# gchq/annchor

Hardware: AMD Instinct MI355X
Metric: knn_graph_builds_per_s (1 / Annchor.fit() wall-clock; BASELINE: k-NN graph build time + recall@k) (higher is better)
Workload: dtype int32 bit-vectors (Levenshtein) + f64 (bounds/regression/selection); 1 GPU; load_strings Levenshtein N=1600 n_anchors=15 k=25 p_work=0.12 niters=2; parallelism=one GPU

## Files before the change

annchor_amd/_native.py:

```python
import ctypes
import os

import numpy as np

_HERE = os.path.dirname(os.path.abspath(__file__))
LIB_PATH = os.environ.get("ANNCHOR_HIP_LIB", os.path.join(_HERE, "libannchor_hip.so"))

F_D, F_A, F_SID, F_IJS, F_I_PTR, F_I_IDX, F_FEATURES, F_NCM, F_RA, F_LABELS, F_THRESH, F_PROB, F_CAND, F_NEXT, F_DAD = range(1, 16)
_FIELD_DTYPE = {
    F_D: np.float64, F_A: np.int64, F_SID: np.uint64, F_IJS: np.int64, F_I_PTR: np.int64, F_I_IDX: np.int64,
    F_FEATURES: np.float64, F_NCM: np.uint8, F_RA: np.float64, F_LABELS: np.int64, F_THRESH: np.float64,
    F_PROB: np.float64, F_CAND: np.int64, F_NEXT: np.int64, F_DAD: np.float64,
}

METRIC_LEVENSHTEIN, METRIC_EUCLIDEAN_F32, METRIC_EUCLIDEAN_F64, METRIC_WASSERSTEIN = 1, 2, 3, 4
METRIC_COSINE_F32, METRIC_COSINE_F64 = 5, 6
METRIC_DTW_F32, METRIC_DTW_F64 = 7, 8
METRIC_FRECHET_F32, METRIC_FRECHET_F64 = 9, 10
METRIC_HAUSDORFF_F32, METRIC_HAUSDORFF_F64 = 11, 12
METRIC_ERP_F32, METRIC_ERP_F64 = 13, 14
METRIC_EMD_POINTS_F32, METRIC_EMD_POINTS_F64 = 15, 16
METRIC_JACCARD_TOKENS, METRIC_JACCARD_BITS = 17, 18
METRIC_WEIGHTED_LEVENSHTEIN = 19
METRIC_MSM_F32, METRIC_MSM_F64 = 20, 21
# ... 71 lines not shown
    "annchor_legacy_generate": (ctypes.c_int, [ctypes.c_uint32, _i64]),
    "annchor_legacy_generate_at_next_wait": (ctypes.c_int, [_vp, ctypes.c_uint32, _i64, _i64]),
    "annchor_legacy_choice_ranks": (ctypes.c_int, [ctypes.c_uint32, _vp, _vp, _i32, _vp, _vp]),
    "annchor_legacy_choice_begin": (ctypes.c_int, [ctypes.c_uint32, _vp, _vp, _i32, ctypes.POINTER(_vp)]),
    "annchor_legacy_choice_end": (ctypes.c_int, [_vp, _vp, _vp]),
    "annchor_ols_bins": (ctypes.c_int, [_vp, _vp, _vp, _i64, _i32, _vp, _i32, _vp, _vp, _vp, _vp]),
    "annchor_gather_features": (ctypes.c_int, [_vp, _vp, _i64, _vp]),
    "annchor_evaluate_samples": (ctypes.c_int, [_vp, _vp, _i64, _vp]),
    "annchor_set_samples": (ctypes.c_int, [_vp, _vp, _i64, _vp]),
    "annchor_predict_merge": (ctypes.c_int, [_vp, _vp, _i32, _vp, _vp, _i32, _i32, _vp]),
    "annchor_merge_host_prediction": (ctypes.c_int, [_vp, _vp, _i32, _i32]),
    "annchor_set_labels": (ctypes.c_int, [_vp, _vp]),
    "annchor_select_candidates": (ctypes.c_int, [_vp, _i32, _i32, _vp, _vp, _i32, _i64, _i32,
                                                 ctypes.POINTER(_i64), ctypes.POINTER(_i64)]),
    "annchor_select_prepare": (ctypes.c_int, [_vp, _i32, _i32]),
    "annchor_mark_candidates": (ctypes.c_int, [_vp]),
    "annchor_refine_candidates": (ctypes.c_int, [_vp]),
    "annchor_park_refine": (ctypes.c_int, [_vp, _i32]),
    "annchor_set_refined": (ctypes.c_int, [_vp, _vp, _i64]),
    "annchor_update_bounds": (ctypes.c_int, [_vp]),
    "annchor_update_bounds_prepare": (ctypes.c_int, [_vp]),
    "annchor_overlap_stats": (ctypes.c_int, [_vp, _vp]),
    "annchor_neighbor_graph": (ctypes.c_int, [_vp, _i32, _vp, _vp]),
    "annchor_stream_bind": (ctypes.c_int, [_vp, _vp, _i64, _i32, _i64, _i32]),
    "annchor_stream_anchor_round": (ctypes.c_int, [_vp, _vp, _i32, _i32, ctypes.POINTER(_dbl), ctypes.POINTER(_i64)]),
    "annchor_stream_get_row": (ctypes.c_int, [_vp, _i64, _vp]),
    "annchor_stream_order": (ctypes.c_int, [_vp, _i32] + [ctypes.POINTER(_vp)] * 6 + [ctypes.POINTER(_i64), ctypes.POINTER(_i32),
                                                                                   ctypes.POINTER(_i32)]),
    "annchor_stream_knn": (ctypes.c_int, [_vp, _vp, _vp, _vp, _vp, _vp, _vp, _i64, _i32, _i32, _i32, _i32, _i32, _i32, _dbl, _i32, _i32, _vp,
                                          _vp, _vp, ctypes.POINTER(_i64)]),
# ... 630 lines not shown
        if errs_list is None:
            self._chk(self.lib.annchor_select_candidates(self.h, int(n_neighbors), int(nmin), None, None, int(n_labels), int(n_refine),
                                                         int(lookahead), ctypes.byref(nc), ctypes.byref(nn)))
            return nc.value, nn.value
        ptr = np.zeros(len(errs_list) + 1, dtype=np.int64)
        np.cumsum([len(e) for e in errs_list], out=ptr[1:])
        errs = _c(np.concatenate(errs_list) if len(errs_list) else np.zeros(0), np.float64)
        self._chk(self.lib.annchor_select_candidates(self.h, int(n_neighbors), int(nmin), _ptr(errs), _ptr(ptr),
                                                     len(errs_list), int(n_refine), int(lookahead),
                                                     ctypes.byref(nc), ctypes.byref(nn)))
        return nc.value, nn.value

    def select_prepare(self, n_neighbors, nmin):
        self._chk(self.lib.annchor_select_prepare(self.h, int(n_neighbors), int(nmin)))

    def mark_candidates(self):
        self._chk(self.lib.annchor_mark_candidates(self.h))

    def refine_candidates(self):
        self._chk(self.lib.annchor_refine_candidates(self.h))

    def park_refine(self, action):
        self._chk(self.lib.annchor_park_refine(self.h, int(action)))

    def set_refined(self, exact):
        exact = _c(exact, np.float64)
        self._chk(self.lib.annchor_set_refined(self.h, _ptr(exact), len(exact)))

    def update_bounds(self):
        self._chk(self.lib.annchor_update_bounds(self.h))
# ... 393 lines not shown
```

annchor_amd/csrc/common.h:

```cpp
#pragma once
#include <hip/hip_runtime.h>

#include <cstdint>
#include <cstdio>
#include <cstring>
#include <string>
#include <vector>
#include <chrono>

#include "../../include/annchor_hip.h"

#define ANN_WAVE 64

struct DevBuf {
    void *p = nullptr;
    size_t cap = 0;
    bool in_arena = false;
    template <typename T> T *as() const { return reinterpret_cast<T *>(p); }
};

struct ProfEntry {
    const char *name;
    double ms = 0;
    int64_t launches = 0;
// ... 127 lines not shown

    DevBuf thresh;
    DevBuf cand, next;
    int64_t ncand = 0, nnext = 0;
    bool cand_marked = false;
    DevBuf gl_val, gl_pos, gl_cnt, gl_ncomp, marked, markcount;
    DevBuf gn_state;
    bool sel_prepared = false;
    int sel_k = 0, sel_nmin = 0;
    bool gn_pending = false;
    int gn_round = 0, gn_L = 0;
    DevBuf sel_hist, sel_state, blk_cnt, blk_off;
    DevBuf sel_pass_state;
    DevBuf tie_lists, tie_hist;
    const void *tie_hist_clean = nullptr;
    DevBuf sel2, sel_bufA, sel_bufB, sel_seg;
    const void *sel2_clean = nullptr;
    DevBuf errs, errptr;
    DevBuf ecdf_index;
    DevBuf cptr, cidx, cval;
    DevBuf c16, cbnd;
    DevBuf tmp0, tmp1, tmp2, tmp3;
    DevBuf scan_tmp;

    DevBuf stage_in, stage_out;

    bool prof_on = false;
    int prof_mode = 0;
    std::vector<hipEvent_t> ev_pool;
    std::vector<ProfEntry> prof;
// ... 30 lines not shown

#define ANN_REQUIRE(c, cond, code, ...)    \
    do {                                   \
        if (!(cond)) {                     \
            ann_set_err((c), __VA_ARGS__); \
            return (code);                 \
        }                                  \
    } while (0)

int ann_reserve(annchor_ctx *c, DevBuf &b, size_t bytes);
int ann_arena_init(annchor_ctx *c, int64_t nx);
int ann_prewarm_state(annchor_ctx *c);
void ann_lev_ap_probe(annchor_ctx *c);
size_t ann_sel2_table_bytes();
size_t ann_tie_hist_bytes();
size_t ann_sel_state_bytes();
int ann_h2d(annchor_ctx *c, void *dst, const void *src, size_t bytes);
hipError_t ann_sync(annchor_ctx *c, const char *where);
int ann_dev_alloc(annchor_ctx *c, void **p, size_t want, size_t *got);
void ann_dev_free(annchor_ctx *c, void *p, size_t bytes);
struct Sel2Epilogue;
int ann_kth_async(annchor_ctx *c, const double *vals, const uint8_t *flag, int64_t n, const int64_t *ks, int nk,
                  const unsigned long long **d_prefix, const int **d_unfinished, const Sel2Epilogue *epi = nullptr);
void ann_kth_async_done(annchor_ctx *c);
int ann_d2h(annchor_ctx *c, void *dst, const void *src, size_t bytes);
int ann_d2h_then(annchor_ctx *c, void *dst, const void *src, size_t bytes, int (*then)(annchor_ctx *));
int ann_d2h2(annchor_ctx *c, void *dst1, const void *src1, size_t bytes1, void *dst2, const void *src2, size_t bytes2);

int ann_prof_entry(annchor_ctx *c, const char *name);
struct ProfGroup {
// ... 180 lines not shown
```

annchor_amd/csrc/ctx.hip:

```cpp
#include <cstdarg>
#include <cmath>
#include <cstdlib>

#include "common.h"
#include <algorithm>
#include <chrono>
#include <mutex>

static std::string g_create_err;
void ann_stream_release(annchor_ctx *c);
void ann_enemies_release(annchor_ctx *c);
void ann_draw_forget(annchor_ctx *c);
void ann_comm_release(annchor_ctx *c);
hipError_t ann_comm_guarded_sync(annchor_ctx *c, hipStream_t stream, const char *where);

const char *ann_set_err(annchor_ctx *c, const char *fmt, ...)
{
    char buf[1024];
    va_list ap;
    va_start(ap, fmt);
    vsnprintf(buf, sizeof buf, fmt, ap);
    va_end(ap);
    if (c && c->comm_aborted && c->err.rfind("collective timed out", 0) == 0) return c->err.c_str();
    if (c) c->err = buf; else g_create_err = buf;
// ... 135 lines not shown
    size_t got = 0;
    if ((p = pool_take(c->device, bytes, &got)) != nullptr) bytes = got;
    else if (hipMalloc(&p, bytes) != hipSuccess) { (void)hipGetLastError(); return ANNCHOR_OK; }
    c->arena = (char *)p;
    c->arena_size = bytes;
    c->arena_off = 0;
    return ANNCHOR_OK;
}

int ann_prewarm_state(annchor_ctx *c)
{
    if (!c->arena || c->state_prewarmed) return ANNCHOR_OK;
    const size_t slot_bytes = sizeof(unsigned long long) * 4 * 1024 + 64;
    struct Piece { DevBuf *b; size_t bytes; };
    Piece pieces[] = {{&c->dev_flags, sizeof(int32_t) * 16}, {&c->lev_cursors, 4 * sizeof(int32_t)}, {&c->sel_state, ann_sel_state_bytes()},
                      {&c->sel2, ann_sel2_table_bytes()},    {&c->tie_hist, ann_tie_hist_bytes()},   {&c->lev_ap, slot_bytes}};
    size_t need = 0;
    for (auto &q : pieces) {
        if (q.b->p) return ANNCHOR_OK;
        need += (q.bytes + 255) & ~(size_t)255;
    }
    if (c->arena_off + need > c->arena_size) return ANNCHOR_OK;
    char *first = c->arena + c->arena_off;
    for (auto &q : pieces) ANN_TRY(ann_reserve(c, *q.b, q.bytes));
    ANN_CHECK_HIP(c, hipMemsetAsync(first, 0, need, c->stream));
    c->dev_flags_clean = true;
    c->lev_cursor_epoch = 0;
    c->gn_err_clean = true;
    c->sel2_clean = c->sel2.p;
    c->tie_hist_clean = c->tie_hist.p;
    c->lev_ap_epoch = 0;
    c->state_prewarmed = true;
    return ANNCHOR_OK;
}

int ann_h2d(annchor_ctx *c, void *dst, const void *src, size_t bytes)
{
    if (bytes == 0) return ANNCHOR_OK;
    if (c->pin && bytes <= annchor_ctx::PIN_SLOT_BYTES) {
        const int sl = c->pin_next;
        c->pin_next = (sl + 1) % annchor_ctx::PIN_SLOTS;
        if (c->pin_busy[sl]) ANN_CHECK_HIP(c, hipEventSynchronize(c->pin_ev[sl]));
        unsigned char *slot = c->pin + (size_t)sl * annchor_ctx::PIN_SLOT_BYTES;
        memcpy(slot, src, bytes);
        ANN_CHECK_HIP(c, hipMemcpyAsync(dst, slot, bytes, hipMemcpyHostToDevice, c->stream));
// ... 1157 lines not shown
```

annchor_amd/csrc/select.hip:

```cpp
#include "common.h"
#include "rowsel.h"
#include "selstate.h"

__global__ __launch_bounds__(ROW_THREADS) void k_row_thresh(const int64_t *__restrict__ Iptr, RowSrc src, uint32_t k,
                                                           double *__restrict__ thresh, int cap)
{
    __shared__ RowSelShared sh;
    __shared__ RowCand rc;
    extern __shared__ __attribute__((aligned(16))) unsigned char dyn_rt[];
    uint64_t *keys = reinterpret_cast<uint64_t *>(dyn_rt);
    const int64_t i = row_of_block(gridDim.x);
    const int64_t b = Iptr[i];
    const int len = (int)(Iptr[i + 1] - b);
    if (len <= 0) { if (threadIdx.x == 0) thresh[i] = -INFINITY; return; }
    const RowView rv = row_view(src, i, b);
    const uint32_t kk = k >= (uint32_t)len ? (uint32_t)len - 1 : k;
    {
        const int cnt = row_candidates(rc, len, (int)kk + 1, [&](int s) { return row_key_asc(rv.val(s)); }, [](int) { return true; },
                                       [](int, uint64_t, bool) {});
        const int cnts = cnt > (int)kk ? row_cand_shrink(rc, cnt, (int)kk + 1, src.shrink_min) : -1;
        if (cnts > (int)kk) {
            for (int e = threadIdx.x; e < cnts; e += ROW_THREADS) {
                const uint64_t ke = rc.key[e];
                uint32_t less = 0, leq = 0;
// ... 490 lines not shown
    const int k0 = threadIdx.x * per, k1 = min(k0 + per, ix.nb + 1);
    uint32_t mine = 0;
    for (int k = k0; k < k1; ++k) mine += T[k];
    csum[threadIdx.x] = mine;
    __syncthreads();
    if (threadIdx.x == 0) {
        uint32_t run = 0;
        for (int q = 0; q < 256; ++q) { const uint32_t v = csum[q]; csum[q] = run; run += v; }
        index[b] = ix;
    }
    __syncthreads();
    uint32_t run = csum[threadIdx.x];
    for (int k = k0; k < k1; ++k) { run += T[k]; T[k] = run; }
}

__global__ __launch_bounds__(256) void k_prob(int64_t n, const int2 *__restrict__ ij, const double *__restrict__ thresh,
                                             const double *__restrict__ RA, const uint8_t *__restrict__ ncm,
                                             const uint8_t *__restrict__ label, const double *__restrict__ errs,
                                             const int64_t *__restrict__ errptr, int nlabels, int lds_cap_entries,
                                             double *__restrict__ prob, int stream, const EcdfIndex *__restrict__ index,
                                             const uint32_t *__restrict__ table)
{
    extern __shared__ __attribute__((aligned(16))) unsigned char dyn[];
    double *le = reinterpret_cast<double *>(dyn);
    __shared__ int64_t lptr[257];
    __shared__ EcdfIndex lix[256];
    for (int t = threadIdx.x; t <= nlabels; t += blockDim.x) lptr[t] = errptr[t];
    if (index)
        for (int t = threadIdx.x; t < nlabels; t += blockDim.x) lix[t] = index[t];
    __syncthreads();
    const bool errs_in_lds = lptr[nlabels] <= (int64_t)lds_cap_entries;
    if (errs_in_lds) {
        const int64_t tot = lptr[nlabels];
        for (int64_t t = threadIdx.x; t < tot; t += blockDim.x) le[t] = errs[t];
        __syncthreads();
    }
    const double *E = errs_in_lds ? le : errs;
    constexpr int PI = 8;
    const int64_t stride = (int64_t)gridDim.x * blockDim.x * PI;
    for (int64_t p0 = (int64_t)blockIdx.x * blockDim.x * PI + threadIdx.x; p0 < n; p0 += stride) {
        uint8_t m[PI], lbv[PI];
        int2 q[PI];
        double ra[PI];
#pragma unroll
        for (int e = 0; e < PI; ++e) {
            const int64_t p = p0 + (int64_t)e * blockDim.x;
            const bool in = p < n;
            const int64_t pc = in ? p : 0;
            m[e] = ann_load(ncm + pc, stream);
            const long long qq = ann_load(reinterpret_cast<const long long *>(ij) + pc, stream);
            q[e] = make_int2((int)(qq & 0xffffffffll), (int)(qq >> 32));
// ... 19 lines not shown
                hi[e] = b[e] + (int32_t)t1;
                lo[e] = b[e] + (int32_t)t0;
            }
            busy |= lo[e] < hi[e];
        }
        while (busy) {
            busy = false;
#pragma unroll
            for (int e = 0; e < PI; ++e)
                if (lo[e] < hi[e]) {
                    const int32_t mid = (lo[e] + hi[e]) >> 1;
                    if (E[mid] < pv[e]) lo[e] = mid + 1; else hi[e] = mid;
                    busy |= lo[e] < hi[e];
                }
        }
#pragma unroll
        for (int e = 0; e < PI; ++e) {
            const int64_t p = p0 + (int64_t)e * blockDim.x;
            if (p >= n) continue;
            double pr = -1.0;
            if (m[e]) {
                if ((int)lbv[e] < nlabels) {
                    const int32_t len = (int32_t)lptr[lbv[e] + 1] - b[e];
                    pr = (double)(lo[e] - b[e]) / (double)len;
                } else {
                    pr = 0.0;
                }
            }
            ann_store(prob + p, pr, stream);
        }
    }
}

#define CP_THREADS 256
#define CP_ITEMS 8
#define CP_SUBTILE (CP_THREADS * CP_ITEMS)
static inline int cp_nsub(int64_t n) { return n >= (16ll << 20) ? 4 : 1; }


#define TIE_CAP 65536

__host__ __device__ __forceinline__ unsigned long long ann_tie_scramble(int64_t p)
{
    return ((unsigned long long)p * 0x9E3779B97F4A7C15ull) >> 11;
}

// ... 34 lines not shown
#pragma unroll
    for (int off = 32; off > 0; off >>= 1) {
        g1 += __shfl_xor(g1, off); g5 += __shfl_xor(g5, off); n1 += __shfl_xor(n1, off); n5 += __shfl_xor(n5, off);
    }
    if ((threadIdx.x & 63) == 0) { atomicAdd(&acc[0], g1); atomicAdd(&acc[1], g5); atomicAdd(&acc[2], n1); atomicAdd(&acc[3], n5); }
    __syncthreads();
    for (int t = threadIdx.x; t < 2 * TIE_BINS; t += 256) {
        const uint32_t c = (&h[0][0])[t];
        if (c) atomicAdd(&ghist[t], c);
    }
    if (threadIdx.x == 0) {
        if (acc[0]) atomicAdd((unsigned long long *)&cs->tie_gt1, acc[0]);
        if (acc[1]) atomicAdd((unsigned long long *)&cs->tie_gt5, acc[1]);
        if (acc[2]) atomicAdd((unsigned long long *)&cs->tie_n1, acc[2]);
        if (acc[3]) atomicAdd((unsigned long long *)&cs->tie_n5, acc[3]);
    }
}

__global__ __launch_bounds__(1024) void k_tie_pick(CutState *__restrict__ cs, uint32_t *__restrict__ ghist)
{
    __shared__ unsigned long long wsum[16];
    const int lane = threadIdx.x & 63, wave = threadIdx.x >> 6;
    for (int q = 0; q < 2; ++q) {
        const bool all = q == 0 ? cs->all1 : cs->all5;
        const long long cnt = q == 0 ? cs->tie_n1 : cs->tie_n5;
        const long long e = q == 0 ? cs->K1 - cs->tie_gt1 : cs->K5 - cs->tie_gt5;
        uint32_t *h = ghist + q * TIE_BINS;
        constexpr int PER = TIE_BINS / 1024;
        unsigned long long c[PER], mine = 0;
#pragma unroll
// ... 467 lines not shown
        for (int q = 0; q < GN_BATCH; ++q, ++round)
            k_gn_round<<<ann_blocks(nx * 64, 256), 256, 0, c->stream>>>(
                nx, nmin, L, Lw, c->gl_val.as<double>(), oth, twin, c->gl_cnt.as<int32_t>(), c->gl_ncomp.as<int32_t>(),
                masks[round & 1], masks[(round + 1) & 1], mout[round % 3], mout[(round + 1) % 3], mout[(round + 2) % 3],
                changed + q, gn_err_ptr(c));
    }
    k_gn_apply<<<ann_blocks(nx * L, 256), 256, 0, c->stream>>>(nx, L, Lw, c->gl_pos.as<int32_t>(), c->gl_cnt.as<int32_t>(),
                                                              masks[round & 1], c->RA.as<double>());
    ANN_CHECK_HIP(c, hipGetLastError());
    c->gn_pending = false;
    return ANNCHOR_OK;
}

size_t ann_tie_hist_bytes() { return sizeof(uint32_t) * 2 * TIE_BINS; }

extern "C" int annchor_select_prepare(annchor_ctx *c, int32_t n_neighbors, int32_t nmin)
{
    if (!c) return ANNCHOR_EINVAL;
    ANN_REQUIRE(c, c->have_RA, ANNCHOR_EINVAL, "RefineApprox not initialised");
    ANN_REQUIRE(c, n_neighbors >= 1 && nmin >= 0, ANNCHOR_EINVAL, "bad selection parameters");
    ANN_CHECK_HIP(c, hipSetDevice(c->device));
    ANN_TRY(select_stage_a(c, n_neighbors, nmin));
    c->sel_prepared = true; c->sel_k = n_neighbors; c->sel_nmin = nmin;
    return ANNCHOR_OK;
}

extern "C" int annchor_select_candidates(annchor_ctx *c, int32_t n_neighbors, int32_t nmin, const double *errs,
                                         const int64_t *err_ptr, int32_t nlabels, int64_t n_refine, int32_t lookahead,
                                         int64_t *n_cand, int64_t *n_next)
{
// ... 9 lines not shown
            ANN_REQUIRE(c, err_ptr[b + 1] > err_ptr[b], ANNCHOR_ESTATE, "error bin %d has no samples", b);
    ANN_CHECK_HIP(c, hipSetDevice(c->device));
    const int64_t n = c->n, nx = c->nx;
    if (!(c->sel_prepared && c->sel_k == n_neighbors && c->sel_nmin == nmin)) ANN_TRY(select_stage_a(c, n_neighbors, nmin));
    c->sel_prepared = false;
    ANN_TRY(select_stage_finish(c));
    (void)nx;
    const int64_t nerr = dev_errs ? 2 * c->nsamp + 64 : err_ptr[nlabels];
    if (!dev_errs) {
        ANN_TRY(ann_reserve(c, c->errs, sizeof(double) * (size_t)nerr));
        ANN_TRY(ann_reserve(c, c->errptr, sizeof(int64_t) * (size_t)(MAXBINS > nlabels ? MAXBINS + 1 : nlabels + 1)));
        ANN_TRY(ann_h2d(c, c->errs.p, errs, sizeof(double) * (size_t)nerr));
        ANN_TRY(ann_h2d(c, c->errptr.p, err_ptr, sizeof(int64_t) * (size_t)(nlabels + 1)));
        c->errs_on_device = false; c->model_cache_valid = false;
    }
    {
        const int64_t lds_entries = dev_errs ? c->nsamp + 64 : nerr;
        const int in_lds = lds_entries * 8 <= 60 * 1024;
        const size_t dyn = in_lds ? (size_t)lds_entries * 8 : 0;
        int blocks = min(ann_blocks(n, 256 * 8), c->prop.multiProcessorCount * 8);
        ProfScope ps(c, "ecdf_probability", (double)n * 26.0);
        static const long long index_min = getenv("ANNCHOR_ECDF_INDEX_MIN") ? atoll(getenv("ANNCHOR_ECDF_INDEX_MIN")) : (4ll << 20);
        EcdfIndex *index = nullptr;
        uint32_t *table = nullptr;
        if (n >= index_min && nlabels > 0 && nerr > 0 && nerr < (1ll << 29)) {
            const size_t idx_bytes = (sizeof(EcdfIndex) * (size_t)nlabels + 15) & ~(size_t)15;
            ANN_TRY(ann_reserve(c, c->ecdf_index, idx_bytes + sizeof(uint32_t) * (size_t)(2 * nerr + nlabels + 1)));
            index = c->ecdf_index.as<EcdfIndex>();
            table = reinterpret_cast<uint32_t *>(c->ecdf_index.as<char>() + idx_bytes);
            k_ecdf_index<<<nlabels, 256, 0, c->stream>>>(c->errs.as<double>(), c->errptr.as<int64_t>(), index, table);
        }
        k_prob<<<blocks, 256, dyn, c->stream>>>(n, c->ij.as<int2>(), c->thresh.as<double>(), c->RA.as<double>(),
                                               c->ncm.as<uint8_t>(), c->label.as<uint8_t>(), c->errs.as<double>(),
                                               c->errptr.as<int64_t>(), nlabels, in_lds ? (int)lds_entries : 0, c->prob.as<double>(), n >= ANN_STREAM_MIN_PAIRS,
                                               index, table);
    }
    ANN_CHECK_HIP(c, hipGetLastError());
    int64_t n_unc = 0;
    ANN_TRY(annchor_count_uncomputed(c, &n_unc));
    CutState cs;
    memset(&cs, 0, sizeof cs);
    cs.K1 = n_refine;
    cs.K5 = n_refine * (int64_t)lookahead;
    cs.all1 = n_refine >= n_unc;
    cs.all5 = cs.all1 || cs.K5 >= n_unc;
    cs.t1 = cs.t5 = INFINITY;
    const unsigned long long *d_cut_prefix = nullptr;
    const int *d_cut_unfinished = nullptr;
    int64_t cut_ks[2];
    int cut_nk = 0;
// ... 8 lines not shown
    if (cs.all1) cs.t1 = -1.0;
    if (cs.all5) cs.t5 = -1.0;
    if (n_refine == 0) { cs.all1 = cs.all5 = 0; cs.t1 = cs.t5 = INFINITY; cs.K1 = cs.K5 = 0; }
    const int nsub = cp_nsub(n);
    const int nb = ann_blocks(n, (int64_t)CP_SUBTILE * nsub);
    ANN_TRY(ann_reserve(c, c->sel_state, SEL_STATE_BYTES));
    ANN_TRY(ann_reserve(c, c->blk_cnt, sizeof(uint32_t) * 4 * (size_t)nb));
    ANN_TRY(ann_reserve(c, c->blk_off, sizeof(int64_t) * 4 * (size_t)nb));
    const int64_t maxc = cs.all1 ? n_unc : cs.K1, maxn = cs.all5 ? n_unc : cs.K5;
    ANN_TRY(ann_reserve(c, c->cand, sizeof(int32_t) * (size_t)(maxc + 1)));
    ANN_TRY(ann_reserve(c, c->next, sizeof(int32_t) * (size_t)(maxn + 1)));
    cs.rk1 = cs.rk5 = ~0ull;
    if (n_refine > 0 && !(cs.all1 && cs.all5)) {
        if (!cs.all1) cut_ks[cut_nk++] = n_unc - cs.K1;
        if (!cs.all5) cut_ks[cut_nk++] = n_unc - cs.K5;
        if (!getenv("ANNCHOR_CUT_WAIT")) {
            Sel2Epilogue ep;
            memset(&ep, 0, sizeof ep);
            ep.kind = 2; ep.cs = c->sel_state.as<CutState>(); ep.cs_init = cs; ep.need1 = !cs.all1; ep.need5 = !cs.all5;
            ep.force_redo = getenv("ANNCHOR_CUT_FORCE_REDO") ? 1 : 0;
            ANN_TRY(ann_kth_async(c, c->prob.as<double>(), c->ncm.as<uint8_t>(), n, cut_ks, cut_nk, &d_cut_prefix, &d_cut_unfinished, &ep));
        }
        if (!d_cut_prefix) ANN_TRY(cut_values_waiting());
    }
    const CutState cs_in = cs;
    if (!d_cut_prefix) ANN_TRY(ann_h2d(c, c->sel_state.p, &cs, sizeof cs));
    const bool ties = n_refine > 0 && !(cs.all1 && cs.all5);
    ANN_TRY(ann_reserve(c, c->tie_lists, sizeof(unsigned long long) * 2 * TIE_CAP));
    unsigned long long *tl1 = c->tie_lists.as<unsigned long long>(), *tl5 = tl1 + TIE_CAP;
    auto split = [&]() {
        ProfScope ps(c, "topk_split_compact", (double)n * 16.0 + (double)(maxc + maxn) * 4.0);
        k_cut_count<<<nb, CP_THREADS, 0, c->stream>>>(c->prob.as<double>(), c->RA.as<double>(), n, c->sel_state.as<CutState>(),
                                                     c->blk_cnt.as<uint32_t>(), nsub);
        k_cut_scan<<<1, CS_THREADS, 0, c->stream>>>(c->blk_cnt.as<uint32_t>(), nb, c->sel_state.as<CutState>(), c->blk_off.as<int64_t>());
        k_cut_emit<<<nb, CP_THREADS, 0, c->stream>>>(c->prob.as<double>(), c->RA.as<double>(), n, c->sel_state.as<CutState>(),
                                                    c->blk_off.as<int64_t>(), c->cand.as<int32_t>(), c->next.as<int32_t>(), nsub);
    };
    auto tie_groups = [&]() -> int {
        ProfScope ps(c, "topk_tie_groups", (double)n * 8.0);
        const int tb = (int)std::min<int64_t>(ann_blocks(n, 256 * TIE_U), (int64_t)c->prop.multiProcessorCount * 3);
        const char *cap_env = getenv("ANNCHOR_TIE_CAP");
        const long long cap = cap_env ? std::min<long long>(TIE_CAP, std::max<long long>(1, atoll(cap_env))) : TIE_CAP;
        ANN_TRY(ann_reserve(c, c->tie_hist, sizeof(uint32_t) * 2 * TIE_BINS));
        if (c->tie_hist_clean != c->tie_hist.p) {
            ANN_CHECK_HIP(c, hipMemsetAsync(c->tie_hist.p, 0, sizeof(uint32_t) * 2 * TIE_BINS, c->stream));
            c->tie_hist_clean = c->tie_hist.p;
        }
        k_tie_hist<<<tb, 256, 0, c->stream>>>(c->prob.as<double>(), n, c->sel_state.as<CutState>(), c->tie_hist.as<uint32_t>());
        k_tie_pick<<<1, 1024, 0, c->stream>>>(c->sel_state.as<CutState>(), c->tie_hist.as<uint32_t>());
        k_tie_collect<<<tb, 256, 0, c->stream>>>(c->prob.as<double>(), n, c->sel_state.as<CutState>(), tl1, tl5, cap);
        k_tie_select<<<1, 1024, 0, c->stream>>>(c->sel_state.as<CutState>(), tl1, tl5, cap);
        return ANNCHOR_OK;
    };
    if (ties) ANN_TRY(tie_groups());
    split();
    ANN_CHECK_HIP(c, hipEventRecord(c->call_b, c->stream));
    c->call_timed = true;
    ANN_CHECK_HIP(c, hipGetLastError());
    if (nmin > 0) {
        unsigned char both[SEL_ERR_OFF + 4];
        ANN_TRY(ann_d2h(c, both, c->sel_state.p, sizeof both));
        int32_t e = 0;
        memcpy(&cs, both, sizeof cs);
        memcpy(&e, both + SEL_ERR_OFF, 4);
        c->gn_err_clean = e == 0;
        ANN_REQUIRE(c, e == 0, ANNCHOR_ESTATE, "guarantee_nmin: a row has fewer not-computed candidates than it must refine");
    } else {
        ANN_TRY(ann_d2h(c, &cs, c->sel_state.p, sizeof cs));
    }
    if (d_cut_prefix) {
        ann_kth_async_done(c);
        if (cs.sel_unfinished) {
            cs = cs_in;
            ANN_TRY(cut_values_waiting());
            ANN_TRY(ann_h2d(c, c->sel_state.p, &cs, sizeof cs));
            if (ties) ANN_TRY(tie_groups());
            split();
            ANN_CHECK_HIP(c, hipGetLastError());
            ANN_TRY(ann_d2h(c, &cs, c->sel_state.p, sizeof cs));
        }
    }
    if (cs.tie_overflow) {
        ANN_TRY(ann_reserve(c, c->marked, (size_t)n));
        for (int q = 0; q < 2; ++q) {
            const bool all = q == 0 ? cs.all1 : cs.all5;
            const int64_t cnt = q == 0 ? cs.tie_n1 : cs.tie_n5, e = q == 0 ? cs.K1 - cs.tie_gt1 : cs.K5 - cs.tie_gt5;
            unsigned long long rk = ~0ull;
            if (!all && e < cnt) {
                if (e <= 0) rk = 0ull;
                else {
                    ANN_TRY(ann_reserve(c, c->colT, sizeof(double) * (size_t)n));
// ... 106 lines not shown
```

include/annchor_hip.h:

```cpp
#ifndef ANNCHOR_HIP_H
#define ANNCHOR_HIP_H

#include <stdint.h>

#ifdef __cplusplus
extern "C" {
#endif

typedef struct annchor_ctx annchor_ctx;

enum {
    ANNCHOR_OK = 0,
    ANNCHOR_EINVAL = -1,
    ANNCHOR_EHIP = -2,
    ANNCHOR_ENODEV = -3,
    ANNCHOR_ELIMIT = -4,
    ANNCHOR_ESTATE = -5
};

enum { ANNCHOR_METRIC_NONE = 0, ANNCHOR_METRIC_LEVENSHTEIN = 1, ANNCHOR_METRIC_EUCLIDEAN_F32 = 2,
       ANNCHOR_METRIC_EUCLIDEAN_F64 = 3, ANNCHOR_METRIC_WASSERSTEIN = 4, ANNCHOR_METRIC_COSINE_F32 = 5,
       ANNCHOR_METRIC_COSINE_F64 = 6, ANNCHOR_METRIC_DTW_F32 = 7, ANNCHOR_METRIC_DTW_F64 = 8,
       ANNCHOR_METRIC_FRECHET_F32 = 9, ANNCHOR_METRIC_FRECHET_F64 = 10, ANNCHOR_METRIC_HAUSDORFF_F32 = 11,
       ANNCHOR_METRIC_HAUSDORFF_F64 = 12, ANNCHOR_METRIC_ERP_F32 = 13, ANNCHOR_METRIC_ERP_F64 = 14,
// ... 132 lines not shown
                                     uint32_t seed, int64_t *n_out, int32_t *taken);
int annchor_legacy_choice_ranks_device(annchor_ctx *ctx, uint32_t seed, const int64_t *counts, const int64_t *want, int32_t nbins,
                                       int64_t *ranks_out, int32_t *taken);
int annchor_download_samples(annchor_ctx *ctx, int64_t *positions, double *feats, double *sample_y, double *sample_predict);
int annchor_fit_regression_device(annchor_ctx *ctx, const double *bins, int32_t nbins, int32_t first_iteration, int32_t is_metric);
int annchor_fit_errors_device(annchor_ctx *ctx);
int annchor_model_download(annchor_ctx *ctx, double *W, double *c, int32_t *status, int64_t *err_ptr, int32_t *flags );
int annchor_errors_download(annchor_ctx *ctx, double *errs, int64_t n_errs);
int annchor_model_download_with_errors(annchor_ctx *ctx, double *W, double *c, int32_t *status, int64_t *err_ptr, int32_t *flags ,
                                       double *errs, int64_t errs_cap, int64_t *n_errs);

int annchor_select_candidates(annchor_ctx *ctx, int32_t n_neighbors, int32_t nmin, const double *errs,
                              const int64_t *err_ptr, int32_t nlabels, int64_t n_refine,
                              int32_t lookahead, int64_t *n_cand, int64_t *n_next);
int annchor_select_prepare(annchor_ctx *ctx, int32_t n_neighbors, int32_t nmin);
int annchor_mark_candidates(annchor_ctx *ctx);
int annchor_refine_candidates(annchor_ctx *ctx);
int annchor_lev_persist_state(int set);

int annchor_park_refine(annchor_ctx *ctx, int32_t action);
int annchor_set_refined(annchor_ctx *ctx, const double *exact, int64_t n_cand);

int annchor_update_bounds(annchor_ctx *ctx);
int annchor_update_bounds_prepare(annchor_ctx *ctx);
int annchor_overlap_stats(annchor_ctx *ctx, int64_t *out);

int annchor_neighbor_graph(annchor_ctx *ctx, int32_t n_neighbors, int64_t *ng_idx, double *ng_dist);

int annchor_stream_bind(annchor_ctx *ctx, const float *X, int64_t n_local, int32_t dim, int64_t global_base,
                        int32_t x_on_device);
// ... 107 lines not shown
```

Baseline: 388.1 graphs/s.

## Derive probability cut thresholds from a fused per-key count table

The probability kernel now builds a per-block shared-memory histogram over the discrete (label, ECDF rank) keys that every probability value maps to, and merges it into a small global table. A single-block kernel then finds the k-th largest cut values and tie-group counts from this table. This replaces the separate async k-th selection pass over all pair probabilities, and a reduced-pass tie histogram follows it. It adds atomic work and LDS pressure to k_prob and falls back to the old path when the table overflows or its totals do not match.

```diff
diff --git a/annchor_amd/_native.py b/annchor_amd/_native.py
--- a/annchor_amd/_native.py
+++ b/annchor_amd/_native.py
@@ -109,6 +109,7 @@
     "annchor_select_candidates": (ctypes.c_int, [_vp, _i32, _i32, _vp, _vp, _i32, _i64, _i32,
                                                  ctypes.POINTER(_i64), ctypes.POINTER(_i64)]),
     "annchor_select_prepare": (ctypes.c_int, [_vp, _i32, _i32]),
+    "annchor_cut_stats": (ctypes.c_int, [_vp, ctypes.POINTER(_i64), ctypes.POINTER(_i64)]),
     "annchor_mark_candidates": (ctypes.c_int, [_vp]),
     "annchor_refine_candidates": (ctypes.c_int, [_vp]),
     "annchor_park_refine": (ctypes.c_int, [_vp, _i32]),
@@ -769,6 +770,11 @@
     def select_prepare(self, n_neighbors, nmin):
         self._chk(self.lib.annchor_select_prepare(self.h, int(n_neighbors), int(nmin)))
 
+    def cut_stats(self):
+        t, f = _i64(), _i64()
+        self._chk(self.lib.annchor_cut_stats(self.h, ctypes.byref(t), ctypes.byref(f)))
+        return t.value, f.value
+
     def mark_candidates(self):
         self._chk(self.lib.annchor_mark_candidates(self.h))
 
diff --git a/annchor_amd/csrc/common.h b/annchor_amd/csrc/common.h
--- a/annchor_amd/csrc/common.h
+++ b/annchor_amd/csrc/common.h
@@ -165,6 +165,9 @@
     DevBuf sel_pass_state;
     DevBuf tie_lists, tie_hist;
     const void *tie_hist_clean = nullptr;
+    DevBuf cut_tab;
+    const void *cut_tab_clean = nullptr;
+    int64_t cut_stat_table = 0, cut_stat_fallback = 0;
     DevBuf sel2, sel_bufA, sel_bufB, sel_seg;
     const void *sel2_clean = nullptr;
     DevBuf errs, errptr;
@@ -225,6 +228,7 @@
 void ann_lev_ap_probe(annchor_ctx *c);
 size_t ann_sel2_table_bytes();
 size_t ann_tie_hist_bytes();
+size_t ann_cut_tab_bytes();
 size_t ann_sel_state_bytes();
 int ann_h2d(annchor_ctx *c, void *dst, const void *src, size_t bytes);
 hipError_t ann_sync(annchor_ctx *c, const char *where);
diff --git a/annchor_amd/csrc/ctx.hip b/annchor_amd/csrc/ctx.hip
--- a/annchor_amd/csrc/ctx.hip
+++ b/annchor_amd/csrc/ctx.hip
@@ -173,7 +173,8 @@
     const size_t slot_bytes = sizeof(unsigned long long) * 4 * 1024 + 64;
     struct Piece { DevBuf *b; size_t bytes; };
     Piece pieces[] = {{&c->dev_flags, sizeof(int32_t) * 16}, {&c->lev_cursors, 4 * sizeof(int32_t)}, {&c->sel_state, ann_sel_state_bytes()},
-                      {&c->sel2, ann_sel2_table_bytes()},    {&c->tie_hist, ann_tie_hist_bytes()},   {&c->lev_ap, slot_bytes}};
+                      {&c->sel2, ann_sel2_table_bytes()},    {&c->tie_hist, ann_tie_hist_bytes()},   {&c->lev_ap, slot_bytes},
+                      {&c->cut_tab, ann_cut_tab_bytes()}};
     size_t need = 0;
     for (auto &q : pieces) {
         if (q.b->p) return ANNCHOR_OK;
@@ -188,6 +189,7 @@
     c->gn_err_clean = true;
     c->sel2_clean = c->sel2.p;
     c->tie_hist_clean = c->tie_hist.p;
+    c->cut_tab_clean = c->cut_tab.p;
     c->lev_ap_epoch = 0;
     c->state_prewarmed = true;
     return ANNCHOR_OK;
diff --git a/annchor_amd/csrc/select.hip b/annchor_amd/csrc/select.hip
--- a/annchor_amd/csrc/select.hip
+++ b/annchor_amd/csrc/select.hip
@@ -528,15 +528,35 @@
     for (int k = k0; k < k1; ++k) { run += T[k]; T[k] = run; }
 }
 
+#define CUT_KEYS 8192
+#define CUT_TAB_MAX_PAIRS (16ll << 20)
+size_t ann_cut_tab_bytes() { return sizeof(uint32_t) * CUT_KEYS; }
+
+__device__ __forceinline__ void cut_tab_add(uint32_t *kh, int32_t g, bool on)
+{
+#pragma unroll
+    for (int r = 0; r < 2; ++r) {
+        const unsigned long long live = __ballot(on);
+        if (!live) return;
+        const int lead = __ffsll(live) - 1;
+        const int32_t gk = __builtin_amdgcn_readlane(g, lead);
+        const unsigned long long same = __ballot(on && g == gk);
+        if ((int)(threadIdx.x & 63) == lead) atomicAdd(&kh[gk], (uint32_t)__popcll(same));
+        on = on && g != gk;
+    }
+    if (on) atomicAdd(&kh[g], 1u);
+}
+
 __global__ __launch_bounds__(256) void k_prob(int64_t n, const int2 *__restrict__ ij, const double *__restrict__ thresh,
                                              const double *__restrict__ RA, const uint8_t *__restrict__ ncm,
                                              const uint8_t *__restrict__ label, const double *__restrict__ errs,
                                              const int64_t *__restrict__ errptr, int nlabels, int lds_cap_entries,
                                              double *__restrict__ prob, int stream, const EcdfIndex *__restrict__ index,
-                                             const uint32_t *__restrict__ table)
+                                             const uint32_t *__restrict__ table, uint32_t *__restrict__ cut_tab, int tab_cap)
 {
     extern __shared__ __attribute__((aligned(16))) unsigned char dyn[];
     double *le = reinterpret_cast<double *>(dyn);
+    uint32_t *kh = reinterpret_cast<uint32_t *>(le + lds_cap_entries);
     __shared__ int64_t lptr[257];
     __shared__ EcdfIndex lix[256];
     for (int t = threadIdx.x; t <= nlabels; t += blockDim.x) lptr[t] = errptr[t];
@@ -544,11 +564,14 @@
         for (int t = threadIdx.x; t < nlabels; t += blockDim.x) lix[t] = index[t];
     __syncthreads();
     const bool errs_in_lds = lptr[nlabels] <= (int64_t)lds_cap_entries;
+    const bool counting = cut_tab && lptr[nlabels] + nlabels + 1 <= (int64_t)tab_cap;
+    const int32_t nkeys = counting ? (int32_t)lptr[nlabels] + nlabels + 1 : 0;
+    for (int t = threadIdx.x; t < nkeys; t += blockDim.x) kh[t] = 0;
     if (errs_in_lds) {
         const int64_t tot = lptr[nlabels];
         for (int64_t t = threadIdx.x; t < tot; t += blockDim.x) le[t] = errs[t];
-        __syncthreads();
-    }
+    }
+    __syncthreads();
     const double *E = errs_in_lds ? le : errs;
     constexpr int PI = 8;
     const int64_t stride = (int64_t)gridDim.x * blockDim.x * PI;
@@ -598,6 +621,11 @@
                     busy |= lo[e] < hi[e];
                 }
         }
+        if (counting) {
+#pragma unroll
+            for (int e = 0; e < PI; ++e)
+                cut_tab_add(kh, (int)lbv[e] < nlabels ? lo[e] + (int32_t)lbv[e] : nkeys - 1, m[e] != 0);
+        }
 #pragma unroll
         for (int e = 0; e < PI; ++e) {
             const int64_t p = p0 + (int64_t)e * blockDim.x;
@@ -614,6 +642,152 @@
             ann_store(prob + p, pr, stream);
         }
     }
+    if (counting) {
+        __syncthreads();
+        for (int t = threadIdx.x; t < nkeys; t += blockDim.x) {
+            const uint32_t cnt = kh[t];
+            if (cnt) atomicAdd(&cut_tab[t], cnt);
+        }
+    }
+}
+
+#define CV_THREADS 1024
+#define CV_PER (CUT_KEYS / CV_THREADS)
+#define CV_BUCKETS 4096
+#define CV_MEMBERS 1024
+__global__ __launch_bounds__(CV_THREADS) void k_tie_cut_values(uint32_t *__restrict__ tab, const int64_t *__restrict__ errptr,
+                                                              int nlabels, int tab_cap, long long n_unc, CutState *__restrict__ cs,
+                                                              CutState init, int need1, int need5, int force_redo)
+{
+    __shared__ long long base[257];
+    __shared__ uint32_t bh[CV_BUCKETS];
+    __shared__ unsigned long long mkey[2][CV_MEMBERS];
+    __shared__ uint32_t mcnt[2][CV_MEMBERS], mnum[2];
+    __shared__ unsigned long long wsum[CV_THREADS / 64], total_s, tkey_s[2];
+    __shared__ long long kin_s[2], gt_s[2], grp_s[2];
+    __shared__ int bucket_s[2], bad_s;
+    const int lane = threadIdx.x & 63, wave = threadIdx.x >> 6;
+    for (int t = threadIdx.x; t <= nlabels; t += CV_THREADS) base[t] = errptr[t] + t;
+    for (int t = threadIdx.x; t < CV_BUCKETS; t += CV_THREADS) bh[t] = 0;
+    if (threadIdx.x == 0) { total_s = 0; bad_s = 0; mnum[0] = mnum[1] = 0; bucket_s[0] = bucket_s[1] = -1; }
+    __syncthreads();
+    const long long S = base[nlabels] + 1;
+    const bool need = need1 || need5;
+    if (S > tab_cap) {
+        if (threadIdx.x == 0) { init.sel_unfinished = need ? 1 : 0; *cs = init; }
+        return;
+    }
+    auto bucket_of = [](unsigned long long kk) -> int {
+        const int b = (int)(__longlong_as_double((long long)kk) * (double)CV_BUCKETS);
+        return b < CV_BUCKETS ? b : CV_BUCKETS - 1;
+    };
+    unsigned long long key[CV_PER];
+    uint32_t cnt[CV_PER];
+    unsigned long long mine = 0;
+    bool bad = false;
+#pragma unroll
+    for (int j = 0; j < CV_PER; ++j) {
+        const int g = threadIdx.x + j * CV_THREADS;
+        key[j] = 0; cnt[j] = 0;
+        if (g < (int)S) {
+            cnt[j] = tab[g];
+            if (cnt[j]) tab[g] = 0;
+            int lo = 0, hi = nlabels;
+            while (lo < hi) { const int mid = (lo + hi + 1) >> 1; if (base[mid] <= g) lo = mid; else hi = mid - 1; }
+            double v = 0.0;
+            if (lo < nlabels) {
+                const int32_t rank = g - (int32_t)base[lo], len = (int32_t)(base[lo + 1] - base[lo]) - 1;
+                if (len > 0) v = (double)rank / (double)len; else bad |= cnt[j] != 0;
+            }
+            key[j] = (unsigned long long)__double_as_longlong(v);
+            mine += cnt[j];
+            if (cnt[j]) atomicAdd(&bh[bucket_of(key[j])], cnt[j]);
+        }
+    }
+#pragma unroll
+    for (int off = 32; off > 0; off >>= 1) mine += __shfl_xor(mine, off);
+    if (lane == 0 && mine) atomicAdd(&total_s, mine);
+    if (bad) bad_s = 1;
+    __syncthreads();
+    if (bad_s || (long long)total_s != n_unc) {
+        if (threadIdx.x == 0) { init.sel_unfinished = need ? 1 : 0; *cs = init; }
+        return;
+    }
+    if (need) {
+        constexpr int BPT = CV_BUCKETS / CV_THREADS;
+        unsigned long long c[BPT], own = 0;
+#pragma unroll
+        for (int j = 0; j < BPT; ++j) { c[j] = bh[CV_BUCKETS - 1 - (threadIdx.x * BPT + j)]; own += c[j]; }
+        unsigned long long inc = own;
+#pragma unroll
+        for (int off = 1; off < 64; off <<= 1) { const unsigned long long up = __shfl_up(inc, off); if (lane >= off) inc += up; }
+        if (lane == 63) wsum[wave] = inc;
+        __syncthreads();
+        unsigned long long before = inc - own;
+        for (int w2 = 0; w2 < wave; ++w2) before += wsum[w2];
+        for (int q = 0; q < 2; ++q) {
+            if (!(q == 0 ? need1 : need5)) continue;
+            const long long K = q == 0 ? init.K1 : init.K5;
+            long long acc = (long long)before;
+            if (acc < K && K <= acc + (long long)own) {
+#pragma unroll
+                for (int j = 0; j < BPT; ++j) {
+                    if (acc < K && K <= acc + (long long)c[j]) { bucket_s[q] = CV_BUCKETS - 1 - (threadIdx.x * BPT + j); kin_s[q] = K - acc; }
+                    acc += (long long)c[j];
+                }
+            }
+        }
+        __syncthreads();
+        const int b1 = bucket_s[0], b5 = bucket_s[1];
+#pragma unroll
+        for (int j = 0; j < CV_PER; ++j) {
+            if (!cnt[j]) continue;
+            const int b = bucket_of(key[j]);
+            if (b == b1) { const uint32_t o = atomicAdd(&mnum[0], 1u); if (o < CV_MEMBERS) { mkey[0][o] = key[j]; mcnt[0][o] = cnt[j]; } }
+            if (b == b5) { const uint32_t o = atomicAdd(&mnum[1], 1u); if (o < CV_MEMBERS) { mkey[1][o] = key[j]; mcnt[1][o] = cnt[j]; } }
+        }
+        __syncthreads();
+        if (mnum[0] > CV_MEMBERS || mnum[1] > CV_MEMBERS) {
+            if (threadIdx.x == 0) { init.sel_unfinished = 1; *cs = init; }
+            return;
+        }
+        for (int q = 0; q < 2; ++q) {
+            const int m = (int)mnum[q];
+            if (bucket_s[q] < 0 || (int)threadIdx.x >= m) continue;
+            const unsigned long long ke = mkey[q][threadIdx.x];
+            long long above = 0, eq = 0;
+            for (int o = 0; o < m; ++o) {
+                const unsigned long long ko = mkey[q][o];
+                const long long co = (long long)mcnt[q][o];
+                above += ko > ke ? co : 0;
+                eq += ko == ke ? co : 0;
+            }
+            const long long kin = kin_s[q];
+            if (above < kin && kin <= above + eq) {
+                tkey_s[q] = ke;
+                gt_s[q] = (q == 0 ? init.K1 : init.K5) - kin + above;
+                grp_s[q] = eq;
+            }
+        }
+        __syncthreads();
+    }
+    if (threadIdx.x == 0 && !need) *cs = init;
+    if (threadIdx.x == 0 && need) {
+        init.tie_gt1 = init.tie_gt5 = n_unc; init.tie_n1 = init.tie_n5 = 0;
+        if (need1) { init.t1 = __longlong_as_double((long long)tkey_s[0]); init.tie_gt1 = gt_s[0]; init.tie_n1 = grp_s[0]; }
+        if (need5) { init.t5 = __longlong_as_double((long long)tkey_s[1]); init.tie_gt5 = gt_s[1]; init.tie_n5 = grp_s[1]; }
+        for (int q = 0; q < 2; ++q) {
+            const bool all = q == 0 ? init.all1 : init.all5;
+            const long long gcnt = q == 0 ? init.tie_n1 : init.tie_n5;
+            const long long e = q == 0 ? init.K1 - init.tie_gt1 : init.K5 - init.tie_gt5;
+            unsigned long long rk = ~0ull;
+            long long bin = -1;
+            if (!all && e < gcnt) { if (e <= 0) rk = 0ull; else bin = -2; }
+            if (q == 0) { init.rk1 = rk; init.tie_bin1 = bin; } else { init.rk5 = rk; init.tie_bin5 = bin; }
+        }
+        init.sel_unfinished = need ? force_redo : 0;
+        *cs = init;
+    }
 }
 
 #define CP_THREADS 256
@@ -678,6 +852,44 @@
         if (acc[1]) atomicAdd((unsigned long long *)&cs->tie_gt5, acc[1]);
         if (acc[2]) atomicAdd((unsigned long long *)&cs->tie_n1, acc[2]);
         if (acc[3]) atomicAdd((unsigned long long *)&cs->tie_n5, acc[3]);
+    }
+}
+
+#define TIE_SPLIT_STEPS 4
+__global__ __launch_bounds__(256) void k_tie_hist_split(const double *__restrict__ prob, int64_t n, const CutState *__restrict__ cs,
+                                                       uint32_t *__restrict__ ghist )
+{
+    __shared__ uint32_t h[2][TIE_BINS];
+    const bool on1 = cs->tie_bin1 == -2, on5 = cs->tie_bin5 == -2;
+    if (!on1 && !on5) return;
+    for (int t = threadIdx.x; t < TIE_BINS; t += 256) {
+        if (on1) h[0][t] = 0;
+        if (on5) h[1][t] = 0;
+    }
+    __syncthreads();
+    const double t1 = cs->t1, t5 = cs->t5;
+    const int64_t stride = (int64_t)gridDim.x * blockDim.x * TIE_U;
+    for (int64_t p0 = (int64_t)blockIdx.x * blockDim.x * TIE_U + threadIdx.x; p0 < n; p0 += stride) {
+        double v[TIE_U];
+#pragma unroll
+        for (int e = 0; e < TIE_U; ++e) v[e] = ann_ldc(prob, p0 + (int64_t)e * blockDim.x, n);
+#pragma unroll
+        for (int e = 0; e < TIE_U; ++e) {
+            const int64_t p = p0 + (int64_t)e * blockDim.x;
+            if (p >= n || !(v[e] >= 0.0)) continue;
+            const bool m1 = on1 && v[e] == t1, m5 = on5 && v[e] == t5;
+            if (m1 || m5) {
+                const uint32_t bin = (uint32_t)(ann_tie_scramble(p) >> TIE_SHIFT);
+                if (m1) atomicAdd(&h[0][bin], 1u);
+                if (m5) atomicAdd(&h[1][bin], 1u);
+            }
+        }
+    }
+    __syncthreads();
+    for (int t = threadIdx.x; t < TIE_BINS; t += 256) {
+        const uint32_t c1 = on1 ? h[0][t] : 0u, c5 = on5 ? h[1][t] : 0u;
+        if (c1) atomicAdd(&ghist[t], c1);
+        if (c5) atomicAdd(&ghist[TIE_BINS + t], c5);
     }
 }
 
@@ -1175,6 +1387,14 @@
 
 size_t ann_tie_hist_bytes() { return sizeof(uint32_t) * 2 * TIE_BINS; }
 
+extern "C" int annchor_cut_stats(annchor_ctx *c, int64_t *table_calls, int64_t *fallback_calls)
+{
+    if (!c || !table_calls || !fallback_calls) return ANNCHOR_EINVAL;
+    *table_calls = c->cut_stat_table;
+    *fallback_calls = c->cut_stat_fallback;
+    return ANNCHOR_OK;
+}
+
 extern "C" int annchor_select_prepare(annchor_ctx *c, int32_t n_neighbors, int32_t nmin)
 {
     if (!c) return ANNCHOR_EINVAL;
@@ -1214,11 +1434,42 @@
         ANN_TRY(ann_h2d(c, c->errptr.p, err_ptr, sizeof(int64_t) * (size_t)(nlabels + 1)));
         c->errs_on_device = false; c->model_cache_valid = false;
     }
+    bool use_tab = false;
+    int tab_cap = 0;
     {
         const int64_t lds_entries = dev_errs ? c->nsamp + 64 : nerr;
         const int in_lds = lds_entries * 8 <= 60 * 1024;
-        const size_t dyn = in_lds ? (size_t)lds_entries * 8 : 0;
+        const char *cc_env = getenv("ANNCHOR_CUT_COUNTS");
+        if (!(cc_env && atoi(cc_env) == 0) && !getenv("ANNCHOR_CUT_WAIT") && n < CUT_TAB_MAX_PAIRS) {
+            use_tab = lds_entries + nlabels + 1 <= (int64_t)CUT_KEYS;
+            if (!use_tab) c->cut_stat_fallback += 1;
+        }
+        tab_cap = use_tab ? CUT_KEYS : 0;
+        const size_t dyn = (in_lds ? (size_t)lds_entries * 8 : 0) + sizeof(uint32_t) * (size_t)tab_cap;
         int blocks = min(ann_blocks(n, 256 * 8), c->prop.multiProcessorCount * 8);
+        if (use_tab) {
+            ANN_TRY(ann_reserve(c, c->cut_tab, ann_cut_tab_bytes()));
+            if (c->cut_tab_clean != c->cut_tab.p)
+                ANN_CHECK_HIP(c, hipMemsetAsync(c->cut_tab.p, 0, ann_cut_tab_bytes(), c->stream));
+            c->cut_tab_clean = nullptr;
+            ANN_TRY(row_lds_prepare(c, k_prob, dyn));
+            static std::mutex mu;
+            static size_t memo_dyn = ~(size_t)0;
+            static int memo_per_cu = 0;
+            int per_cu = 0;
+            {
+                std::lock_guard<std::mutex> lk(mu);
+                if (memo_dyn != dyn) {
+                    ANN_CHECK_HIP(c, hipOccupancyMaxActiveBlocksPerMultiprocessor(&memo_per_cu, k_prob, 256, dyn));
+                    memo_dyn = dyn;
+                }
+                per_cu = memo_per_cu;
+            }
+            const int slots = min(blocks, c->prop.multiProcessorCount * std::max(per_cu, 1));
+            const int tiles = ann_blocks(n, 256 * 8);
+            const int rounds = (tiles + slots - 1) / slots;
+            blocks = min(slots, (tiles + rounds - 1) / rounds);
+        }
         ProfScope ps(c, "ecdf_probability", (double)n * 26.0);
         static const long long index_min = getenv("ANNCHOR_ECDF_INDEX_MIN") ? atoll(getenv("ANNCHOR_ECDF_INDEX_MIN")) : (4ll << 20);
         EcdfIndex *index = nullptr;
@@ -1233,7 +1484,7 @@
         k_prob<<<blocks, 256, dyn, c->stream>>>(n, c->ij.as<int2>(), c->thresh.as<double>(), c->RA.as<double>(),
                                                c->ncm.as<uint8_t>(), c->label.as<uint8_t>(), c->errs.as<double>(),
                                                c->errptr.as<int64_t>(), nlabels, in_lds ? (int)lds_entries : 0, c->prob.as<double>(), n >= ANN_STREAM_MIN_PAIRS,
-                                               index, table);
+                                               index, table, use_tab ? c->cut_tab.as<uint32_t>() : nullptr, tab_cap);
     }
     ANN_CHECK_HIP(c, hipGetLastError());
     int64_t n_unc = 0;
@@ -1272,17 +1523,17 @@
     if (n_refine > 0 && !(cs.all1 && cs.all5)) {
         if (!cs.all1) cut_ks[cut_nk++] = n_unc - cs.K1;
         if (!cs.all5) cut_ks[cut_nk++] = n_unc - cs.K5;
-        if (!getenv("ANNCHOR_CUT_WAIT")) {
+        if (!use_tab && !getenv("ANNCHOR_CUT_WAIT")) {
             Sel2Epilogue ep;
             memset(&ep, 0, sizeof ep);
             ep.kind = 2; ep.cs = c->sel_state.as<CutState>(); ep.cs_init = cs; ep.need1 = !cs.all1; ep.need5 = !cs.all5;
             ep.force_redo = getenv("ANNCHOR_CUT_FORCE_REDO") ? 1 : 0;
             ANN_TRY(ann_kth_async(c, c->prob.as<double>(), c->ncm.as<uint8_t>(), n, cut_ks, cut_nk, &d_cut_prefix, &d_cut_unfinished, &ep));
         }
-        if (!d_cut_prefix) ANN_TRY(cut_values_waiting());
+        if (!use_tab && !d_cut_prefix) ANN_TRY(cut_values_waiting());
     }
     const CutState cs_in = cs;
-    if (!d_cut_prefix) ANN_TRY(ann_h2d(c, c->sel_state.p, &cs, sizeof cs));
+    if (!use_tab && !d_cut_prefix) ANN_TRY(ann_h2d(c, c->sel_state.p, &cs, sizeof cs));
     const bool ties = n_refine > 0 && !(cs.all1 && cs.all5);
     ANN_TRY(ann_reserve(c, c->tie_lists, sizeof(unsigned long long) * 2 * TIE_CAP));
     unsigned long long *tl1 = c->tie_lists.as<unsigned long long>(), *tl5 = tl1 + TIE_CAP;
@@ -1294,8 +1545,15 @@
         k_cut_emit<<<nb, CP_THREADS, 0, c->stream>>>(c->prob.as<double>(), c->RA.as<double>(), n, c->sel_state.as<CutState>(),
                                                     c->blk_off.as<int64_t>(), c->cand.as<int32_t>(), c->next.as<int32_t>(), nsub);
     };
-    auto tie_groups = [&]() -> int {
+    auto tie_groups = [&](bool from_table) -> int {
         ProfScope ps(c, "topk_tie_groups", (double)n * 8.0);
+        if (from_table) {
+            k_tie_cut_values<<<1, CV_THREADS, 0, c->stream>>>(c->cut_tab.as<uint32_t>(), c->errptr.as<int64_t>(), nlabels, tab_cap, (long long)n_unc,
+                                                             c->sel_state.as<CutState>(), cs, ties && !cs.all1, ties && !cs.all5,
+                                                             getenv("ANNCHOR_CUT_FORCE_REDO") ? 1 : 0);
+            c->cut_tab_clean = c->cut_tab.p;
+            if (!ties) return ANNCHOR_OK;
+        }
         const int tb = (int)std::min<int64_t>(ann_blocks(n, 256 * TIE_U), (int64_t)c->prop.multiProcessorCount * 3);
         const char *cap_env = getenv("ANNCHOR_TIE_CAP");
         const long long cap = cap_env ? std::min<long long>(TIE_CAP, std::max<long long>(1, atoll(cap_env))) : TIE_CAP;
@@ -1304,13 +1562,18 @@
             ANN_CHECK_HIP(c, hipMemsetAsync(c->tie_hist.p, 0, sizeof(uint32_t) * 2 * TIE_BINS, c->stream));
             c->tie_hist_clean = c->tie_hist.p;
         }
-        k_tie_hist<<<tb, 256, 0, c->stream>>>(c->prob.as<double>(), n, c->sel_state.as<CutState>(), c->tie_hist.as<uint32_t>());
+        if (from_table) {
+            const int tbs = (int)std::min<int64_t>(ann_blocks(n, 256 * TIE_U * TIE_SPLIT_STEPS), (int64_t)c->prop.multiProcessorCount * 3);
+            k_tie_hist_split<<<tbs, 256, 0, c->stream>>>(c->prob.as<double>(), n, c->sel_state.as<CutState>(), c->tie_hist.as<uint32_t>());
+        } else {
+            k_tie_hist<<<tb, 256, 0, c->stream>>>(c->prob.as<double>(), n, c->sel_state.as<CutState>(), c->tie_hist.as<uint32_t>());
+        }
         k_tie_pick<<<1, 1024, 0, c->stream>>>(c->sel_state.as<CutState>(), c->tie_hist.as<uint32_t>());
         k_tie_collect<<<tb, 256, 0, c->stream>>>(c->prob.as<double>(), n, c->sel_state.as<CutState>(), tl1, tl5, cap);
         k_tie_select<<<1, 1024, 0, c->stream>>>(c->sel_state.as<CutState>(), tl1, tl5, cap);
         return ANNCHOR_OK;
     };
-    if (ties) ANN_TRY(tie_groups());
+    if (ties || use_tab) ANN_TRY(tie_groups(use_tab));
     split();
     ANN_CHECK_HIP(c, hipEventRecord(c->call_b, c->stream));
     c->call_timed = true;
@@ -1326,13 +1589,14 @@
     } else {
         ANN_TRY(ann_d2h(c, &cs, c->sel_state.p, sizeof cs));
     }
-    if (d_cut_prefix) {
-        ann_kth_async_done(c);
+    if (d_cut_prefix || use_tab) {
+        if (d_cut_prefix) ann_kth_async_done(c);
+        if (use_tab) (cs.sel_unfinished ? c->cut_stat_fallback : c->cut_stat_table) += 1;
         if (cs.sel_unfinished) {
             cs = cs_in;
             ANN_TRY(cut_values_waiting());
             ANN_TRY(ann_h2d(c, c->sel_state.p, &cs, sizeof cs));
-            if (ties) ANN_TRY(tie_groups());
+            if (ties) ANN_TRY(tie_groups(false));
             split();
             ANN_CHECK_HIP(c, hipGetLastError());
             ANN_TRY(ann_d2h(c, &cs, c->sel_state.p, sizeof cs));
diff --git a/include/annchor_hip.h b/include/annchor_hip.h
--- a/include/annchor_hip.h
+++ b/include/annchor_hip.h
@@ -170,6 +170,7 @@
                               const int64_t *err_ptr, int32_t nlabels, int64_t n_refine,
                               int32_t lookahead, int64_t *n_cand, int64_t *n_next);
 int annchor_select_prepare(annchor_ctx *ctx, int32_t n_neighbors, int32_t nmin);
+int annchor_cut_stats(annchor_ctx *ctx, int64_t *table_calls, int64_t *fallback_calls);
 int annchor_mark_candidates(annchor_ctx *ctx);
 int annchor_refine_candidates(annchor_ctx *ctx);
 int annchor_lev_persist_state(int set);
```

Result: slower. 367.6 graphs/s (-5.3%).
